# GuildOfWeavers/distaff

Hardware: NVIDIA H100
Metric: prove ms for 2^20-step trace (default 120-bit ProofOptions) (lower is better)
Workload: dtype u128 (128-bit prime field) + u32 (blake3)

## Files before the change

distaff_b200/csrc/air.cu:

```cuda
#define DG_MUL_CALL 1
#include "air.h"
#include "air_constants.h"

namespace dg {

__constant__ fe c_sponge_mds[16], c_sponge_inv_mds[16], c_hasher_mds[36], c_hasher_inv_mds[36];

void air_upload_constants(Context &c) {
    if (c.air_consts) return;
    auto conv = [](const unsigned long long (*t)[2], int n, std::vector<fe> &out) {
        out.resize(n);
        for (int i = 0; i < n; i++) out[i] = fe_make(t[i][0], t[i][1]);
    };
    std::vector<fe> v;
    conv(DG_SPONGE_MDS, 16, v);      DG_CUDA(cudaMemcpyToSymbol(c_sponge_mds, v.data(), 16 * sizeof(fe)));
    conv(DG_SPONGE_INV_MDS, 16, v);  DG_CUDA(cudaMemcpyToSymbol(c_sponge_inv_mds, v.data(), 16 * sizeof(fe)));
    conv(DG_HASHER_MDS, 36, v);      DG_CUDA(cudaMemcpyToSymbol(c_hasher_mds, v.data(), 36 * sizeof(fe)));
    conv(DG_HASHER_INV_MDS, 36, v);  DG_CUDA(cudaMemcpyToSymbol(c_hasher_inv_mds, v.data(), 36 * sizeof(fe)));
    c.air_consts = true;
}

__device__ __forceinline__ fe tw_pow(const TwiddleRef &t, unsigned long long e) {
    unsigned ee = (unsigned)(e & (unsigned long long)t.mask);
    return fe_mul(t.lo[ee & ((1u << t.lo_bits) - 1u)], t.hi[ee >> t.lo_bits]);
}

#ifdef DG_AIR_NOSYNC
#define DG_STEP()
#else
#define DG_STEP() __syncthreads()
#endif

template <int W>
__device__ __forceinline__ void matvec(const fe *m, fe *s) {
    fe r[W];
#pragma unroll
    for (int i = 0; i < W; i++) {
        r[i] = fe_dot<W>(m + i * W, s);
        DG_STEP();
    }
#pragma unroll
    for (int i = 0; i < W; i++) s[i] = r[i];
}

#define ONE fe_make(1, 0)
#define ZERO fe_make(0, 0)
__device__ __forceinline__ fe bnot(fe v) { return fe_sub(ONE, v); }
__device__ __forceinline__ fe is_bin(fe v) { return fe_sub(fe_sqr(v), v); }

enum { G2 = 0, G3 = 1, G4 = 2, G6 = 3, G7 = 4, G8 = 5 };

struct Acc {
    fe_wide res;
    fe adj[6];
    const fe *cA, *cB;
    bool nonzero, first;
    __device__ __forceinline__ void fold(int idx, int group, fe v) {
        if (first) { wide_set(res, DG_MUL_WIDE(v, cA[idx])); first = false; }
        else wide_add(res, DG_MUL_WIDE(v, cA[idx]));
        adj[group] = fe_add(adj[group], fe_mul(v, cB[idx]));
        nonzero = nonzero || !fe_is_zero(v);
    }
};

template <int BLOCK, int MIN_BLOCKS>
__global__ void __launch_bounds__(BLOCK, MIN_BLOCKS) constraint_eval_kernel(const AirParams P) {
    const unsigned long long n = 1ULL << P.log_n;
    const unsigned long long total = n * (unsigned long long)P.num_c8;
    unsigned long long gid = (unsigned long long)blockIdx.x * blockDim.x + threadIdx.x;
    const bool live = gid < total;
    if (!live) gid = total - 1;
    const unsigned long long c8_local = gid >> P.log_n, k = gid & (n - 1);
    const unsigned long long c8 = c8_local + P.c8_base;
    const unsigned long long s = (k << 3) + c8;
    const int stride = 1 << (P.log_blowup - 3);
    const unsigned long long N = P.col_stride;
    const unsigned long long lde_index = s * (unsigned long long)stride;
    const fe *cur_p = P.ext + (c8_local * stride) * n + k;
    const fe *nxt_p = P.ext + (c8_local * stride) * n + ((k + 1) & (n - 1));
    const unsigned long long out_idx = (c8_local << P.log_n) + k;

    const int cl = P.cl, ll = P.ll, sl = P.sl;
    const int ctx_off = 15, loop_off = 15 + P.ctx_depth, stk_off = 15 + P.ctx_depth + P.loop_depth;

    fe cur_dec[15], nxt_dec[15];
    fe c_ctx[16], n_ctx[16], c_loop[8], n_loop[8], o[32], nw[32];
    {
        for (int j = 0; j < 15; j++) cur_dec[j] = cur_p[(unsigned long long)j * N];
        for (int j = 0; j < P.ctx_depth; j++) c_ctx[j] = cur_p[(unsigned long long)(ctx_off + j) * N];
        for (int j = 0; j < P.loop_depth; j++) c_loop[j] = cur_p[(unsigned long long)(loop_off + j) * N];
        for (int j = 0; j < P.stack_depth; j++) o[j] = cur_p[(unsigned long long)(stk_off + j) * N];
        for (int j = P.ctx_depth; j < cl; j++) c_ctx[j] = ZERO;
        for (int j = P.loop_depth; j < ll; j++) c_loop[j] = ZERO;
        for (int j = P.stack_depth; j < sl; j++) o[j] = ZERO;
        for (int j = 0; j < 15; j++) nxt_dec[j] = nxt_p[(unsigned long long)j * N];
        for (int j = 0; j < P.ctx_depth; j++) n_ctx[j] = nxt_p[(unsigned long long)(ctx_off + j) * N];
        for (int j = P.ctx_depth; j < cl; j++) n_ctx[j] = ZERO;
        for (int j = 0; j < P.loop_depth; j++) n_loop[j] = nxt_p[(unsigned long long)(loop_off + j) * N];
        for (int j = P.loop_depth; j < ll; j++) n_loop[j] = ZERO;
        for (int j = 0; j < P.stack_depth; j++) nw[j] = nxt_p[(unsigned long long)(stk_off + j) * N];
        for (int j = P.stack_depth; j < sl; j++) nw[j] = ZERO;
    }

    DG_STEP();
    const fe op_counter = cur_dec[0];
    const fe *sp = cur_dec + 1, *cf = cur_dec + 5, *ld = cur_dec + 8, *hd = cur_dec + 13;
    const fe *nsp = nxt_dec + 1, *ncf = nxt_dec + 5;
    fe cff[8], ldf[32], hdf[4];
    {
        fe a3 = fe_mul(cf[0], cf[1]);
        fe a1 = fe_sub(cf[0], a3), a2 = fe_sub(cf[1], a3), a0 = fe_sub(bnot(cf[0]), a2);
        cff[4] = fe_mul(a0, cf[2]); cff[5] = fe_mul(a1, cf[2]); cff[6] = fe_mul(a2, cf[2]); cff[7] = fe_mul(a3, cf[2]);
        cff[0] = fe_sub(a0, cff[4]); cff[1] = fe_sub(a1, cff[5]); cff[2] = fe_sub(a2, cff[6]); cff[3] = fe_sub(a3, cff[7]);
    }
    fe hdf_raw0;
    {
        hdf[3] = fe_mul(hd[0], hd[1]);
        hdf[1] = fe_sub(hd[0], hdf[3]); hdf[2] = fe_sub(hd[1], hdf[3]); hdf[0] = fe_sub(bnot(hd[0]), hdf[2]);
        hdf_raw0 = hdf[0];
        hdf[0] = fe_mul(hdf[0], ld[0]);
    }
    fe next_void;
    {
        fe a3 = fe_mul(ncf[0], ncf[1]);
        next_void = fe_mul(a3, ncf[2]);
    }

    Acc acc;
    acc.first = true;
#pragma unroll
    for (int g = 0; g < 6; g++) acc.adj[g] = ZERO;
    acc.cA = P.coefA; acc.cB = P.coefB; acc.nonzero = false;

    const fe *per = P.per_override ? P.per_override : P.periodic + (s & 127ULL) * 23;

    DG_STEP();
    {
        fe cf_sum = ZERO, ld_prod = ONE, hd_prod = ONE;
#pragma unroll
        for (int i = 0; i < 3; i++) { acc.fold(i, G2, is_bin(cf[i])); cf_sum = fe_add(cf_sum, cf[i]); }
#pragma unroll
        for (int i = 0; i < 5; i++) { acc.fold(3 + i, G2, is_bin(ld[i])); ld_prod = fe_mul(ld_prod, ld[i]); }
#pragma unroll
        for (int i = 0; i < 2; i++) { acc.fold(8 + i, G2, is_bin(hd[i])); hd_prod = fe_mul(hd_prod, hd[i]); }
        fe is_hacc = cff[0];
        fe hacc_t = fe_mul(fe_add(op_counter, ONE), is_hacc);
        fe rest_t = fe_mul(op_counter, bnot(is_hacc));
        acc.fold(10, G3, fe_sub(fe_add(hacc_t, rest_t), nxt_dec[0]));
        acc.fold(11, G8, fe_mul(op_counter, fe_mul(bnot(ld_prod), bnot(hd_prod))));
        acc.fold(12, G8, fe_mul(cf_sum, bnot(fe_mul(ld_prod, hd_prod))));
        acc.fold(13, G6, fe_mul(cff[7], bnot(next_void)));
        fe prefix = fe_add(fe_add(cff[1], cff[4]), fe_add(cff[5], cff[6]));
        fe align = fe_mul(prefix, per[8 + 1]);
        align = fe_add(align, fe_mul(fe_add(cff[2], cff[3]), per[8 + 0]));
        align = fe_add(align, fe_mul(hdf[0], per[8 + 2]));
        acc.fold(14, G4, align);
    }

    DG_STEP();
    {
        fe r_sp[4], r_img;
        {
            fe f = cff[0];
            fe op_value = fe_mul(nw[0], hdf[0]);
            fe os[4], ns[4];
#pragma unroll
            for (int i = 0; i < 4; i++) os[i] = fe_cube(fe_add(sp[i], per[i]));
            DG_STEP();
            matvec<4>(c_sponge_mds, os);
            fe opc = ld[0];
            opc = fe_add(opc, fe_mul_small(ld[1], 2)); opc = fe_add(opc, fe_mul_small(ld[2], 4));
            opc = fe_add(opc, fe_mul_small(ld[3], 8)); opc = fe_add(opc, fe_mul_small(ld[4], 16));
            opc = fe_add(opc, fe_mul_small(hd[0], 32)); opc = fe_add(opc, fe_mul_small(hd[1], 64));
            os[0] = fe_add(os[0], opc);
            os[1] = fe_add(os[1], op_value);
#pragma unroll
            for (int i = 0; i < 4; i++) ns[i] = nsp[i];
            matvec<4>(c_sponge_inv_mds, ns);
#pragma unroll
            for (int i = 0; i < 4; i++) ns[i] = fe_sub(fe_cube(ns[i]), per[4 + i]);
#pragma unroll
            for (int i = 0; i < 4; i++) r_sp[i] = fe_mul(f, fe_sub(os[i], ns[i]));
        }
        DG_STEP();
        {
            fe fclr = fe_add(fe_add(cff[1], cff[4]), cff[5]);
#pragma unroll
            for (int i = 0; i < 4; i++) r_sp[i] = fe_add(r_sp[i], fe_mul(fclr, nsp[i]));
        }
        DG_STEP();
        {
            fe ft = cff[2], ff = cff[3], fb = fe_add(ft, ff);
            r_sp[0] = fe_add(r_sp[0], fe_mul(fb, fe_sub(c_ctx[0], nsp[0])));
            r_sp[1] = fe_add(r_sp[1], fe_mul(ft, fe_sub(sp[0], nsp[1])));
            r_sp[2] = fe_add(r_sp[2], fe_mul(ff, fe_sub(sp[0], nsp[2])));
            r_sp[3] = fe_add(r_sp[3], fe_mul(fb, nsp[3]));
        }
        {
            fe fk = fe_add(cff[6], cff[7]);
#pragma unroll
            for (int i = 0; i < 4; i++) r_sp[i] = fe_add(r_sp[i], fe_mul(fk, fe_sub(sp[i], nsp[i])));
        }
        acc.fold(15, G6, r_sp[0]); acc.fold(16, G7, r_sp[1]); acc.fold(17, G6, r_sp[2]); acc.fold(18, G6, r_sp[3]);
        r_img = fe_mul(fe_add(cff[5], cff[6]), fe_sub(sp[0], c_loop[0]));
        acc.fold(19, G4, r_img);

        DG_STEP();
        {
            fe f_push = fe_add(cff[1], cff[4]), f_pop = fe_add(cff[2], cff[3]), f_copy = fe_add(fe_add(cff[5], cff[6]), cff[7]);
            for (int i = 0; i < cl; i++) {
                fe v = fe_mul(f_copy, fe_sub(c_ctx[i], n_ctx[i]));
                if (i == 0) v = fe_add(v, fe_mul(f_push, fe_sub(sp[0], n_ctx[0])));
// ... 215 lines not shown
    }
    if (live) P.t_ev[out_idx] = t_res;
}

template <int BLOCK, int MIN_BLOCKS, bool STAGE_DEC, bool WIDE_SLOTS>
__global__ void __launch_bounds__(BLOCK, MIN_BLOCKS) constraint_eval_smem_kernel(const AirParams P) {
    extern __shared__ __align__(16) unsigned char air_smem[];
    fe *s_rows = reinterpret_cast<fe *>(air_smem);
    constexpr int PITCH = BLOCK + 1;
    const int tid = threadIdx.x;
    const unsigned long long n = 1ULL << P.log_n;
    const unsigned long long total = n * (unsigned long long)P.num_c8;
    unsigned long long gid = (unsigned long long)blockIdx.x * blockDim.x + threadIdx.x;
    const bool live = gid < total;
    if (!live) gid = total - 1;
    const unsigned long long c8_local = gid >> P.log_n, k = gid & (n - 1);
    const unsigned long long c8 = c8_local + P.c8_base;
    const unsigned long long s = (k << 3) + c8;
    const int stride = 1 << (P.log_blowup - 3);
    const unsigned long long N = P.col_stride;
    const unsigned long long lde_index = s * (unsigned long long)stride;
    const fe *cur_p = P.ext + (c8_local * stride) * n + k;
    const fe *nxt_p = P.ext + (c8_local * stride) * n + ((k + 1) & (n - 1));
    const unsigned long long out_idx = (c8_local << P.log_n) + k;

    const int cl = P.cl, ll = P.ll, sl = P.sl;
    const int ctx_off = 15, loop_off = 15 + P.ctx_depth, stk_off = 15 + P.ctx_depth + P.loop_depth;

    constexpr int S0 = STAGE_DEC ? 0 : 15;
    {
        const int staged = P.w - S0;
        for (int j = 0; j < staged; j++) s_rows[j * PITCH + tid] = cur_p[(unsigned long long)(S0 + j) * N];
        if (tid < staged) {
            const unsigned long long gl = (unsigned long long)blockIdx.x * BLOCK + (BLOCK - 1);
            const unsigned long long cl8 = gl >> P.log_n, kl = gl & (n - 1);
            s_rows[tid * PITCH + BLOCK] = P.ext[(unsigned long long)(S0 + tid) * N + (cl8 * stride) * n + ((kl + 1) & (n - 1))];
        }
    }
    fe cur_dec[STAGE_DEC ? 1 : 15], nxt_dec[STAGE_DEC ? 1 : 15];
    if constexpr (!STAGE_DEC) {
#pragma unroll
        for (int j = 0; j < 15; j++) { cur_dec[j] = cur_p[(unsigned long long)j * N]; nxt_dec[j] = nxt_p[(unsigned long long)j * N]; }
    }
    __syncthreads();
#define DCUR(j) (STAGE_DEC ? s_rows[(j) * PITCH + tid] : cur_dec[STAGE_DEC ? 0 : (j)])
#define DNXT(j) (STAGE_DEC ? s_rows[(j) * PITCH + tid + 1] : nxt_dec[STAGE_DEC ? 0 : (j)])
#define SCOL(col, nx) s_rows[((col) - S0) * PITCH + tid + (nx)]
#define C_CTX(i) (((i) < P.ctx_depth) ? SCOL(ctx_off + (i), 0) : ZERO)
#define N_CTX(i) (((i) < P.ctx_depth) ? SCOL(ctx_off + (i), 1) : ZERO)
#define C_LOOP(i) (((i) < P.loop_depth) ? SCOL(loop_off + (i), 0) : ZERO)
#define N_LOOP(i) (((i) < P.loop_depth) ? SCOL(loop_off + (i), 1) : ZERO)
#define O(i) (((i) < P.stack_depth) ? SCOL(stk_off + (i), 0) : ZERO)
#define NW(i) (((i) < P.stack_depth) ? SCOL(stk_off + (i), 1) : ZERO)

    DG_STEP();
    const fe op_counter = DCUR(0);
#define sp(i) DCUR(1 + (i))
#define cf(i) DCUR(5 + (i))
#define ld(i) DCUR(8 + (i))
#define hd(i) DCUR(13 + (i))
#define nsp(i) DNXT(1 + (i))
#define ncf(i) DNXT(5 + (i))
    fe cff[8], ldf[32], hdf[4];
    {
        fe a3 = fe_mul(cf(0), cf(1));
        fe a1 = fe_sub(cf(0), a3), a2 = fe_sub(cf(1), a3), a0 = fe_sub(bnot(cf(0)), a2);
        cff[4] = fe_mul(a0, cf(2)); cff[5] = fe_mul(a1, cf(2)); cff[6] = fe_mul(a2, cf(2)); cff[7] = fe_mul(a3, cf(2));
        cff[0] = fe_sub(a0, cff[4]); cff[1] = fe_sub(a1, cff[5]); cff[2] = fe_sub(a2, cff[6]); cff[3] = fe_sub(a3, cff[7]);
    }
    fe hdf_raw0;
    {
        hdf[3] = fe_mul(hd(0), hd(1));
        hdf[1] = fe_sub(hd(0), hdf[3]); hdf[2] = fe_sub(hd(1), hdf[3]); hdf[0] = fe_sub(bnot(hd(0)), hdf[2]);
        hdf_raw0 = hdf[0];
        hdf[0] = fe_mul(hdf[0], ld(0));
    }
    fe next_void;
    {
        fe a3 = fe_mul(ncf(0), ncf(1));
        next_void = fe_mul(a3, ncf(2));
    }

    Acc acc;
    acc.first = true;
#pragma unroll
    for (int g = 0; g < 6; g++) acc.adj[g] = ZERO;
    acc.cA = P.coefA; acc.cB = P.coefB; acc.nonzero = false;

    const fe *per = P.per_override ? P.per_override : P.periodic + (s & 127ULL) * 23;

    DG_STEP();
    {
        fe cf_sum = ZERO, ld_prod = ONE, hd_prod = ONE;
#pragma unroll
        for (int i = 0; i < 3; i++) { acc.fold(i, G2, is_bin(cf(i))); cf_sum = fe_add(cf_sum, cf(i)); }
#pragma unroll
        for (int i = 0; i < 5; i++) { acc.fold(3 + i, G2, is_bin(ld(i))); ld_prod = fe_mul(ld_prod, ld(i)); }
#pragma unroll
        for (int i = 0; i < 2; i++) { acc.fold(8 + i, G2, is_bin(hd(i))); hd_prod = fe_mul(hd_prod, hd(i)); }
        fe is_hacc = cff[0];
        fe hacc_t = fe_mul(fe_add(op_counter, ONE), is_hacc);
        fe rest_t = fe_mul(op_counter, bnot(is_hacc));
        acc.fold(10, G3, fe_sub(fe_add(hacc_t, rest_t), DNXT(0)));
        acc.fold(11, G8, fe_mul(op_counter, fe_mul(bnot(ld_prod), bnot(hd_prod))));
        acc.fold(12, G8, fe_mul(cf_sum, bnot(fe_mul(ld_prod, hd_prod))));
        acc.fold(13, G6, fe_mul(cff[7], bnot(next_void)));
        fe prefix = fe_add(fe_add(cff[1], cff[4]), fe_add(cff[5], cff[6]));
        fe align = fe_mul(prefix, per[8 + 1]);
        align = fe_add(align, fe_mul(fe_add(cff[2], cff[3]), per[8 + 0]));
        align = fe_add(align, fe_mul(hdf[0], per[8 + 2]));
        acc.fold(14, G4, align);
    }

    DG_STEP();
    {
        fe r_sp[4], r_img;
        {
            fe f = cff[0];
            fe op_value = fe_mul(NW(0), hdf[0]);
            fe os[4], ns[4];
#pragma unroll
            for (int i = 0; i < 4; i++) os[i] = fe_cube(fe_add(sp(i), per[i]));
            DG_STEP();
            matvec<4>(c_sponge_mds, os);
            fe opc = ld(0);
            opc = fe_add(opc, fe_mul_small(ld(1), 2)); opc = fe_add(opc, fe_mul_small(ld(2), 4));
            opc = fe_add(opc, fe_mul_small(ld(3), 8)); opc = fe_add(opc, fe_mul_small(ld(4), 16));
            opc = fe_add(opc, fe_mul_small(hd(0), 32)); opc = fe_add(opc, fe_mul_small(hd(1), 64));
            os[0] = fe_add(os[0], opc);
            os[1] = fe_add(os[1], op_value);
#pragma unroll
            for (int i = 0; i < 4; i++) ns[i] = nsp(i);
            matvec<4>(c_sponge_inv_mds, ns);
#pragma unroll
            for (int i = 0; i < 4; i++) ns[i] = fe_sub(fe_cube(ns[i]), per[4 + i]);
#pragma unroll
            for (int i = 0; i < 4; i++) r_sp[i] = fe_mul(f, fe_sub(os[i], ns[i]));
        }
        DG_STEP();
        {
            fe fclr = fe_add(fe_add(cff[1], cff[4]), cff[5]);
#pragma unroll
            for (int i = 0; i < 4; i++) r_sp[i] = fe_add(r_sp[i], fe_mul(fclr, nsp(i)));
        }
        DG_STEP();
        {
            fe ft = cff[2], ff = cff[3], fb = fe_add(ft, ff);
            r_sp[0] = fe_add(r_sp[0], fe_mul(fb, fe_sub(C_CTX(0), nsp(0))));
            r_sp[1] = fe_add(r_sp[1], fe_mul(ft, fe_sub(sp(0), nsp(1))));
            r_sp[2] = fe_add(r_sp[2], fe_mul(ff, fe_sub(sp(0), nsp(2))));
            r_sp[3] = fe_add(r_sp[3], fe_mul(fb, nsp(3)));
        }
        {
            fe fk = fe_add(cff[6], cff[7]);
#pragma unroll
            for (int i = 0; i < 4; i++) r_sp[i] = fe_add(r_sp[i], fe_mul(fk, fe_sub(sp(i), nsp(i))));
        }
        acc.fold(15, G6, r_sp[0]); acc.fold(16, G7, r_sp[1]); acc.fold(17, G6, r_sp[2]); acc.fold(18, G6, r_sp[3]);
        r_img = fe_mul(fe_add(cff[5], cff[6]), fe_sub(sp(0), C_LOOP(0)));
        acc.fold(19, G4, r_img);

        DG_STEP();
        {
            fe f_push = fe_add(cff[1], cff[4]), f_pop = fe_add(cff[2], cff[3]), f_copy = fe_add(fe_add(cff[5], cff[6]), cff[7]);
            for (int i = 0; i < cl; i++) {
                fe v = fe_mul(f_copy, fe_sub(C_CTX(i), N_CTX(i)));
                if (i == 0) v = fe_add(v, fe_mul(f_push, fe_sub(sp(0), N_CTX(0))));
// ... 169 lines not shown
            fe c = O(4), nc = bnot(c);
            ev[0] = fe_add(ev[0], fe_mul(f_choose2, fe_sub(NW(0), fe_add(fe_mul(c, O(0)), fe_mul(nc, O(2))))));
            ev[1] = fe_add(ev[1], fe_mul(f_choose2, fe_sub(NW(1), fe_add(fe_mul(c, O(1)), fe_mul(nc, O(3))))));
            ev[0] = fe_add(ev[0], fe_mul(f_cswap2, fe_sub(NW(0), fe_add(fe_mul(c, O(2)), fe_mul(nc, O(0))))));
            ev[1] = fe_add(ev[1], fe_mul(f_cswap2, fe_sub(NW(1), fe_add(fe_mul(c, O(3)), fe_mul(nc, O(1))))));
            ev[2] = fe_add(ev[2], fe_mul(f_cswap2, fe_sub(NW(2), fe_add(fe_mul(c, O(0)), fe_mul(nc, O(2))))));
            ev[3] = fe_add(ev[3], fe_mul(f_cswap2, fe_sub(NW(3), fe_add(fe_mul(c, O(1)), fe_mul(nc, O(3))))));
        }
        DG_STEP();
        {
            fe bit = NW(0);
            ev[0] = fe_add(ev[0], fe_mul(f_binacc, is_bin(bit)));
            ev[1] = fe_add(ev[1], fe_mul(f_binacc, NW(1)));
            ev[2] = fe_add(ev[2], fe_mul(f_binacc, fe_sub(NW(2), fe_mul_small(O(2), 2))));
            ev[3] = fe_add(ev[3], fe_mul(f_binacc, fe_sub(NW(3), fe_add(O(3), fe_mul(bit, O(2))))));
        }
        DG_STEP();
        {
            fe xb = NW(1), yb = NW(2), not_set = NW(3);
            fe bit_gt = fe_mul(xb, bnot(yb)), bit_lt = fe_mul(yb, bnot(xb));
            fe gt = fe_add(O(4), fe_mul(bit_gt, not_set)), lt = fe_add(O(5), fe_mul(bit_lt, not_set));
            fe p2 = O(0);
            fe x_acc = fe_add(O(7), fe_mul(xb, p2)), y_acc = fe_add(O(6), fe_mul(yb, p2));
            fe nsc = fe_mul(bnot(O(5)), bnot(O(4)));
            ev[0] = fe_add(ev[0], fe_mul(f_cmp, is_bin(xb)));
            ev[1] = fe_add(ev[1], fe_mul(f_cmp, is_bin(yb)));
            ev[2] = fe_add(ev[2], fe_mul(f_cmp, fe_sub(NW(4), gt)));
            ev[3] = fe_add(ev[3], fe_mul(f_cmp, fe_sub(NW(5), lt)));
            ev[4] = fe_add(ev[4], fe_mul(f_cmp, fe_sub(NW(6), y_acc)));
            ev[5] = fe_add(ev[5], fe_mul(f_cmp, fe_sub(NW(7), x_acc)));
            ev[6] = fe_add(ev[6], fe_mul(f_cmp, fe_sub(not_set, nsc)));
            ev[7] = fe_add(ev[7], fe_mul(f_cmp, fe_sub(fe_mul_small(NW(0), 2), p2)));
        }
        DG_STEP();
        {
            fe os[6], ns[6];
#pragma unroll
            for (int q = 0; q < 6; q++) os[q] = fe_cube(fe_add(O(q), per[11 + q]));
            matvec<6>(c_hasher_mds, os);
#pragma unroll
            for (int q = 0; q < 6; q++) ns[q] = NW(q);
            matvec<6>(c_hasher_inv_mds, ns);
#pragma unroll
            for (int q = 0; q < 6; q++) ns[q] = fe_sub(fe_cube(ns[q]), per[11 + 6 + q]);
#pragma unroll
            for (int q = 0; q < 6; q++) ev[q] = fe_add(ev[q], fe_mul(f_rescr, fe_sub(ns[q], os[q])));
        }
#pragma unroll
        for (int i = 0; i < 8; i++)
            if (i < P.stack_depth) acc.fold(base + 2 + i, G7, ev[i]);
    }

    DG_STEP();
    fe t_res = DG_REDUCE_WIDE(acc.res);
#pragma unroll
    for (int g = 0; g < 6; g++) t_res = fe_add(t_res, fe_mul(acc.adj[g], P.xpow_override ? P.xpow_override[g] : tw_pow(P.twN, lde_index * P.inc[g])));
    if (!P.verify_mode && c8 == 0 && k != n - 1) {
        if (acc.nonzero && live) atomicExch(P.violation, (unsigned)(k + 1));
        t_res = ZERO;
    }
    if (live) P.t_ev[out_idx] = t_res;
}

#undef DCUR
#undef DNXT
#undef SCOL
#undef C_CTX
#undef N_CTX
#undef C_LOOP
#undef N_LOOP
#undef O
#undef NW
#undef sp
#undef cf
#undef ld
#undef hd
#undef nsp
#undef ncf

void launch_constraint_eval(Context &c, const AirParams &P) {
    air_upload_constants(c);
    const unsigned long long E = (unsigned long long)P.num_c8 << P.log_n;
    static int variant = -1;
    if (variant < 0) { const char *e = getenv("DG_AIR_CFG"); variant = e ? atoi(e) : 7; }
#define DG_AIR_LAUNCH(BLOCK, MINB) constraint_eval_kernel<BLOCK, MINB><<<(unsigned)((E + BLOCK - 1) / BLOCK), BLOCK, 0, c.stream>>>(P)
#define DG_AIR_LAUNCH_SMEM(BLOCK, MINB, DEC, WIDE)                                                                                         \
    do {                                                                                                                             \
        const size_t smem = (size_t)(P.w - ((DEC) ? 0 : 15)) * (BLOCK + 1) * sizeof(fe);                                             \
        auto k = constraint_eval_smem_kernel<BLOCK, MINB, DEC, WIDE>;                                                                      \
        set_func_smem(c, (const void *)k, smem);                                                                                     \
        k<<<(unsigned)(E / BLOCK), BLOCK, smem, c.stream>>>(P);                                                                      \
    } while (0)
    int v = variant;
    const unsigned long long n = 1ULL << P.log_n;
    if (v < 5 || v > 7) v = 1;
    if (v >= 5 && (n < 128 || (size_t)P.w * 129 * sizeof(fe) > 200 * 1024)) v = 1;
    switch (v) {
        case 5: DG_AIR_LAUNCH_SMEM(128, 4, false, false); break;
        case 6: DG_AIR_LAUNCH_SMEM(128, 4, true, false); break;
        case 7: DG_AIR_LAUNCH_SMEM(128, 4, true, true); break;
        default: DG_AIR_LAUNCH(128, 4); break;
    }
    c.launches++;
    DG_CUDA(cudaGetLastError());
}

}
```

distaff_b200/csrc/air.h:

```cpp
#pragma once
#include "common.cuh"

namespace dg {

struct AirParams {
    int w, ctx_depth, loop_depth, stack_depth;
    int cl, ll, sl;
    int log_n, log_blowup;
    const fe *ext;
    unsigned long long col_stride;
    int c8_base, num_c8;
    fe *t_ev;
    const fe *periodic;
    const fe *coefA, *coefB;
    TwiddleRef twN;
    unsigned long long inc[6];
    unsigned *violation;
    int verify_mode;
    const fe *per_override;
    const fe *xpow_override;
};

void launch_constraint_eval(Context &c, const AirParams &P);

}
```

Before: 95.79.

## Split constraint evaluation into three phase kernels with smaller staged column sets

Replaces the single monolithic constraint-evaluation kernel with three sequential phase kernels: decoder/sponge/context/loop, stack shifts and ops, and hasher/comparison. Each phase stages only the columns it needs into shared memory, which lowers per-kernel register pressure and shared memory use and should raise occupancy. Partial sums are accumulated into t_ev across phases. Boundary rows needing cross-phase values go through a temporary ev0 buffer, and wide (unreduced) accumulators are kept for the adjustment groups. The cost is extra launches, re-reading some columns and the output buffer, plus a device allocation per call.

```diff
diff --git a/distaff_b200/csrc/air.cu b/distaff_b200/csrc/air.cu
--- a/distaff_b200/csrc/air.cu
+++ b/distaff_b200/csrc/air.cu
@@ -1,5 +1,5 @@
 #define DG_MUL_CALL 1
-#include "air.h"
+#include "air_eval.cuh"
 #include "air_constants.h"
 
 namespace dg {
@@ -19,49 +19,6 @@
     conv(DG_HASHER_INV_MDS, 36, v);  DG_CUDA(cudaMemcpyToSymbol(c_hasher_inv_mds, v.data(), 36 * sizeof(fe)));
     c.air_consts = true;
 }
-
-__device__ __forceinline__ fe tw_pow(const TwiddleRef &t, unsigned long long e) {
-    unsigned ee = (unsigned)(e & (unsigned long long)t.mask);
-    return fe_mul(t.lo[ee & ((1u << t.lo_bits) - 1u)], t.hi[ee >> t.lo_bits]);
-}
-
-#ifdef DG_AIR_NOSYNC
-#define DG_STEP()
-#else
-#define DG_STEP() __syncthreads()
-#endif
-
-template <int W>
-__device__ __forceinline__ void matvec(const fe *m, fe *s) {
-    fe r[W];
-#pragma unroll
-    for (int i = 0; i < W; i++) {
-        r[i] = fe_dot<W>(m + i * W, s);
-        DG_STEP();
-    }
-#pragma unroll
-    for (int i = 0; i < W; i++) s[i] = r[i];
-}
-
-#define ONE fe_make(1, 0)
-#define ZERO fe_make(0, 0)
-__device__ __forceinline__ fe bnot(fe v) { return fe_sub(ONE, v); }
-__device__ __forceinline__ fe is_bin(fe v) { return fe_sub(fe_sqr(v), v); }
-
-enum { G2 = 0, G3 = 1, G4 = 2, G6 = 3, G7 = 4, G8 = 5 };
-
-struct Acc {
-    fe_wide res;
-    fe adj[6];
-    const fe *cA, *cB;
-    bool nonzero, first;
-    __device__ __forceinline__ void fold(int idx, int group, fe v) {
-        if (first) { wide_set(res, DG_MUL_WIDE(v, cA[idx])); first = false; }
-        else wide_add(res, DG_MUL_WIDE(v, cA[idx]));
-        adj[group] = fe_add(adj[group], fe_mul(v, cB[idx]));
-        nonzero = nonzero || !fe_is_zero(v);
-    }
-};
 
 template <int BLOCK, int MIN_BLOCKS>
 __global__ void __launch_bounds__(BLOCK, MIN_BLOCKS) constraint_eval_kernel(const AirParams P) {
@@ -127,7 +84,7 @@
     }
 
     Acc acc;
-    acc.first = true;
+    acc.first = true; acc.combine = true;
 #pragma unroll
     for (int g = 0; g < 6; g++) acc.adj[g] = ZERO;
     acc.cA = P.coefA; acc.cB = P.coefB; acc.nonzero = false;
@@ -509,7 +466,7 @@
     }
 
     Acc acc;
-    acc.first = true;
+    acc.first = true; acc.combine = true;
 #pragma unroll
     for (int g = 0; g < 6; g++) acc.adj[g] = ZERO;
     acc.cA = P.coefA; acc.cB = P.coefB; acc.nonzero = false;
@@ -845,26 +802,24 @@
     air_upload_constants(c);
     const unsigned long long E = (unsigned long long)P.num_c8 << P.log_n;
     static int variant = -1;
-    if (variant < 0) { const char *e = getenv("DG_AIR_CFG"); variant = e ? atoi(e) : 7; }
-#define DG_AIR_LAUNCH(BLOCK, MINB) constraint_eval_kernel<BLOCK, MINB><<<(unsigned)((E + BLOCK - 1) / BLOCK), BLOCK, 0, c.stream>>>(P)
-#define DG_AIR_LAUNCH_SMEM(BLOCK, MINB, DEC, WIDE)                                                                                         \
-    do {                                                                                                                             \
-        const size_t smem = (size_t)(P.w - ((DEC) ? 0 : 15)) * (BLOCK + 1) * sizeof(fe);                                             \
-        auto k = constraint_eval_smem_kernel<BLOCK, MINB, DEC, WIDE>;                                                                      \
-        set_func_smem(c, (const void *)k, smem);                                                                                     \
-        k<<<(unsigned)(E / BLOCK), BLOCK, smem, c.stream>>>(P);                                                                      \
-    } while (0)
+    if (variant < 0) { const char *e = getenv("DG_AIR_CFG"); variant = e ? atoi(e) : 8; }
     int v = variant;
     const unsigned long long n = 1ULL << P.log_n;
-    if (v < 5 || v > 7) v = 1;
-    if (v >= 5 && (n < 128 || (size_t)P.w * 129 * sizeof(fe) > 200 * 1024)) v = 1;
-    switch (v) {
-        case 5: DG_AIR_LAUNCH_SMEM(128, 4, false, false); break;
-        case 6: DG_AIR_LAUNCH_SMEM(128, 4, true, false); break;
-        case 7: DG_AIR_LAUNCH_SMEM(128, 4, true, true); break;
-        default: DG_AIR_LAUNCH(128, 4); break;
-    }
-    c.launches++;
+    if (v != 7 && v != 8) v = 1;
+    if (v == 7 && (P.verify_mode || n < 128 || (size_t)P.w * 129 * sizeof(fe) > 200 * 1024)) v = 1;
+    if (v == 8 && !constraint_phases_fit(P)) v = 1;
+    if (v == 8) {
+        launch_constraint_phases(c, P);
+    } else if (v == 7) {
+        const size_t smem = (size_t)P.w * 129 * sizeof(fe);
+        auto k = constraint_eval_smem_kernel<128, 4, true, true>;
+        set_func_smem(c, (const void *)k, smem);
+        k<<<(unsigned)(E / 128), 128, smem, c.stream>>>(P);
+        c.launches++;
+    } else {
+        constraint_eval_kernel<128, 4><<<(unsigned)((E + 127) / 128), 128, 0, c.stream>>>(P);
+        c.launches++;
+    }
     DG_CUDA(cudaGetLastError());
 }
 
diff --git a/distaff_b200/csrc/air.h b/distaff_b200/csrc/air.h
--- a/distaff_b200/csrc/air.h
+++ b/distaff_b200/csrc/air.h
@@ -22,5 +22,7 @@
 };
 
 void launch_constraint_eval(Context &c, const AirParams &P);
+bool constraint_phases_fit(const AirParams &P);
+void launch_constraint_phases(Context &c, const AirParams &P);
 
 }
diff --git a/distaff_b200/csrc/air_eval.cuh b/distaff_b200/csrc/air_eval.cuh
--- /dev/null
+++ b/distaff_b200/csrc/air_eval.cuh
@@ -0,0 +1,75 @@
+#pragma once
+#include "air.h"
+
+namespace dg {
+
+extern __constant__ fe c_sponge_mds[16], c_sponge_inv_mds[16], c_hasher_mds[36], c_hasher_inv_mds[36];
+
+__device__ __forceinline__ fe tw_pow(const TwiddleRef &t, unsigned long long e) {
+    unsigned ee = (unsigned)(e & (unsigned long long)t.mask);
+    return fe_mul(t.lo[ee & ((1u << t.lo_bits) - 1u)], t.hi[ee >> t.lo_bits]);
+}
+
+#ifdef DG_AIR_NOSYNC
+#define DG_STEP()
+#else
+#define DG_STEP() __syncthreads()
+#endif
+
+template <int W>
+__device__ __forceinline__ void matvec(const fe *m, fe *s) {
+    fe r[W];
+#pragma unroll
+    for (int i = 0; i < W; i++) {
+        r[i] = fe_dot<W>(m + i * W, s);
+        DG_STEP();
+    }
+#pragma unroll
+    for (int i = 0; i < W; i++) s[i] = r[i];
+}
+
+#define ONE fe_make(1, 0)
+#define ZERO fe_make(0, 0)
+__device__ __forceinline__ fe bnot(fe v) { return fe_sub(ONE, v); }
+__device__ __forceinline__ fe is_bin(fe v) { return fe_sub(fe_sqr(v), v); }
+
+enum { G2 = 0, G3 = 1, G4 = 2, G6 = 3, G7 = 4, G8 = 5 };
+
+struct Acc {
+    fe_wide res;
+    fe adj[6];
+    const fe *cA, *cB;
+    bool nonzero, first, combine;
+    __device__ __forceinline__ void fold(int idx, int group, fe v) {
+        if (combine) {
+            if (first) { wide_set(res, DG_MUL_WIDE(v, cA[idx])); first = false; }
+            else wide_add(res, DG_MUL_WIDE(v, cA[idx]));
+            adj[group] = fe_add(adj[group], fe_mul(v, cB[idx]));
+        }
+        nonzero = nonzero || !fe_is_zero(v);
+    }
+};
+
+struct AccWide {
+    fe_wide res, adj[6];
+    const fe *cA, *cB;
+    bool nonzero, combine;
+    __device__ __forceinline__ void init(const fe *a, const fe *b, bool comb) {
+#pragma unroll
+        for (int i = 0; i < 9; i++) {
+            res.r[i] = 0;
+#pragma unroll
+            for (int g = 0; g < 6; g++) adj[g].r[i] = 0;
+        }
+        cA = a; cB = b; nonzero = false; combine = comb;
+    }
+    __device__ __forceinline__ void fold(int idx, int group, fe v) {
+        if (combine) {
+            wide_add(res, DG_MUL_WIDE(v, cA[idx]));
+            wide_add(adj[group], DG_MUL_WIDE(v, cB[idx]));
+        }
+        nonzero = nonzero || !fe_is_zero(v);
+    }
+};
+
+}
diff --git a/distaff_b200/csrc/air_phase.cu b/distaff_b200/csrc/air_phase.cu
--- /dev/null
+++ b/distaff_b200/csrc/air_phase.cu
@@ -0,0 +1,479 @@
+#define DG_MUL_CALL 1
+#include "air_eval.cuh"
+
+namespace dg {
+
+namespace {
+
+constexpr int PH_BLOCK = 128;
+constexpr int PH_PITCH = PH_BLOCK + 1;
+
+template <int PHASE> struct PhaseCols {
+    static constexpr int a0 = PHASE == 0 ? 0 : PHASE == 1 ? 6 : 13;
+    static constexpr int na = 15 - a0;
+};
+template <int PHASE>
+__host__ __device__ __forceinline__ void phase_range(const AirParams &P, int &b0, int &b1) {
+    const int stk_off = 15 + P.ctx_depth + P.loop_depth;
+    if (PHASE == 0) { b0 = 15; b1 = stk_off + (P.stack_depth > 0 ? 1 : 0); }
+    else if (PHASE == 1) { b0 = stk_off; b1 = P.w; }
+    else { b0 = stk_off; b1 = stk_off + (P.stack_depth < 8 ? P.stack_depth : 8); }
+}
+template <int PHASE>
+size_t phase_smem(const AirParams &P) {
+    int b0, b1;
+    phase_range<PHASE>(P, b0, b1);
+    return (size_t)(PhaseCols<PHASE>::na + b1 - b0) * PH_PITCH * sizeof(fe);
+}
+
+template <int PHASE, int GROUPS>
+__device__ __forceinline__ void phase_finish(const AirParams &P, const AccWide &acc, unsigned long long c8, unsigned long long k, unsigned long long n,
+                                             unsigned long long lde_index, unsigned long long out_idx, bool live) {
+    fe t = ZERO;
+    if (acc.combine) {
+        t = DG_REDUCE_WIDE(acc.res);
+#pragma unroll
+        for (int g = 0; g < 6; g++)
+            if (GROUPS & (1 << g)) t = fe_add(t, fe_mul(DG_REDUCE_WIDE(acc.adj[g]), tw_pow(P.twN, lde_index * P.inc[g])));
+    }
+    if (c8 == 0 && k != n - 1) {
+        if (acc.nonzero && live) atomicExch(P.violation, (unsigned)(k + 1));
+        t = ZERO;
+    }
+    if (live) P.t_ev[out_idx] = PHASE == 0 ? t : fe_add(P.t_ev[out_idx], t);
+}
+
+template <int PHASE, int MINB>
+__global__ void __launch_bounds__(PH_BLOCK, MINB) constraint_phase_kernel(const AirParams P, fe *ev0) {
+    extern __shared__ __align__(16) unsigned char air_smem[];
+    fe *s_rows = reinterpret_cast<fe *>(air_smem);
+    constexpr int BLOCK = PH_BLOCK, PITCH = PH_PITCH;
+    constexpr int A0 = PhaseCols<PHASE>::a0, NA = PhaseCols<PHASE>::na;
+    const int tid = threadIdx.x;
+    const unsigned long long n = 1ULL << P.log_n;
+    const unsigned long long total = n * (unsigned long long)P.num_c8;
+    unsigned long long gid = (unsigned long long)blockIdx.x * blockDim.x + threadIdx.x;
+    const bool live = gid < total;
+    if (!live) gid = total - 1;
+    const unsigned long long c8_local = gid >> P.log_n, k = gid & (n - 1);
+    const unsigned long long c8 = c8_local + P.c8_base;
+    const unsigned long long s = (k << 3) + c8;
+    const int stride = 1 << (P.log_blowup - 3);
+    const unsigned long long N = P.col_stride;
+    const unsigned long long lde_index = s * (unsigned long long)stride;
+    const fe *cur_p = P.ext + (c8_local * stride) * n + k;
+    const unsigned long long out_idx = (c8_local << P.log_n) + k;
+
+    const int cl = P.cl, ll = P.ll;
+    const int ctx_off = 15, loop_off = 15 + P.ctx_depth, stk_off = 15 + P.ctx_depth + P.loop_depth;
+    int B0, B1;
+    phase_range<PHASE>(P, B0, B1);
+    {
+        const int staged = NA + B1 - B0;
+        for (int j = 0; j < staged; j++) {
+            const int col = j < NA ? A0 + j : B0 + (j - NA);
+            s_rows[j * PITCH + tid] = cur_p[(unsigned long long)col * N];
+        }
+        if (tid < staged) {
+            const int col = tid < NA ? A0 + tid : B0 + (tid - NA);
+            const unsigned long long gl = (unsigned long long)blockIdx.x * BLOCK + (BLOCK - 1);
+            const unsigned long long cl8 = gl >> P.log_n, kl = gl & (n - 1);
+            s_rows[tid * PITCH + BLOCK] = P.ext[(unsigned long long)col * N + (cl8 * stride) * n + ((kl + 1) & (n - 1))];
+        }
+    }
+    __syncthreads();
+#define DCUR(j) s_rows[((j) - A0) * PITCH + tid]
+#define DNXT(j) s_rows[((j) - A0) * PITCH + tid + 1]
+#define SCOL(col, nx) s_rows[(NA + (col) - B0) * PITCH + tid + (nx)]
+#define C_CTX(i) (((i) < P.ctx_depth) ? SCOL(ctx_off + (i), 0) : ZERO)
+#define N_CTX(i) (((i) < P.ctx_depth) ? SCOL(ctx_off + (i), 1) : ZERO)
+#define C_LOOP(i) (((i) < P.loop_depth) ? SCOL(loop_off + (i), 0) : ZERO)
+#define N_LOOP(i) (((i) < P.loop_depth) ? SCOL(loop_off + (i), 1) : ZERO)
+#define O(i) (((i) < P.stack_depth) ? SCOL(stk_off + (i), 0) : ZERO)
+#define NW(i) (((i) < P.stack_depth) ? SCOL(stk_off + (i), 1) : ZERO)
+#define sp(i) DCUR(1 + (i))
+#define cf(i) DCUR(5 + (i))
+#define ld(i) DCUR(8 + (i))
+#define hd(i) DCUR(13 + (i))
+#define nsp(i) DNXT(1 + (i))
+#define ncf(i) DNXT(5 + (i))
+
+    AccWide acc;
+    {
+        const unsigned long long k_last = ((unsigned long long)blockIdx.x * BLOCK + (BLOCK - 1)) & (n - 1);
+        acc.init(P.coefA, P.coefB, c8 != 0 || k_last == n - 1);
+    }
+    const fe *per = P.periodic + (s & 127ULL) * 23;
+    const int base = 20 + cl + ll;
+
+    if constexpr (PHASE == 0) {
+        const fe op_counter = DCUR(0);
+        fe cff[8], push_flag, next_void;
+        {
+            fe a3 = fe_mul(cf(0), cf(1));
+            fe a1 = fe_sub(cf(0), a3), a2 = fe_sub(cf(1), a3), a0 = fe_sub(bnot(cf(0)), a2);
+            cff[4] = fe_mul(a0, cf(2)); cff[5] = fe_mul(a1, cf(2)); cff[6] = fe_mul(a2, cf(2)); cff[7] = fe_mul(a3, cf(2));
+            cff[0] = fe_sub(a0, cff[4]); cff[1] = fe_sub(a1, cff[5]); cff[2] = fe_sub(a2, cff[6]); cff[3] = fe_sub(a3, cff[7]);
+        }
+        {
+            fe h3 = fe_mul(hd(0), hd(1));
+            push_flag = fe_mul(fe_sub(bnot(hd(0)), fe_sub(hd(1), h3)), ld(0));
+        }
+        {
+            fe a3 = fe_mul(ncf(0), ncf(1));
+            next_void = fe_mul(a3, ncf(2));
+        }
+        DG_STEP();
+        {
+            fe cf_sum = ZERO, ld_prod = ONE, hd_prod = ONE;
+#pragma unroll
+            for (int i = 0; i < 3; i++) { acc.fold(i, G2, is_bin(cf(i))); cf_sum = fe_add(cf_sum, cf(i)); }
+#pragma unroll
+            for (int i = 0; i < 5; i++) { acc.fold(3 + i, G2, is_bin(ld(i))); ld_prod = fe_mul(ld_prod, ld(i)); }
+#pragma unroll
+            for (int i = 0; i < 2; i++) { acc.fold(8 + i, G2, is_bin(hd(i))); hd_prod = fe_mul(hd_prod, hd(i)); }
+            fe is_hacc = cff[0];
+            fe hacc_t = fe_mul(fe_add(op_counter, ONE), is_hacc);
+            fe rest_t = fe_mul(op_counter, bnot(is_hacc));
+            acc.fold(10, G3, fe_sub(fe_add(hacc_t, rest_t), DNXT(0)));
+            acc.fold(11, G8, fe_mul(op_counter, fe_mul(bnot(ld_prod), bnot(hd_prod))));
+            acc.fold(12, G8, fe_mul(cf_sum, bnot(fe_mul(ld_prod, hd_prod))));
+            acc.fold(13, G6, fe_mul(cff[7], bnot(next_void)));
+            fe prefix = fe_add(fe_add(cff[1], cff[4]), fe_add(cff[5], cff[6]));
+            fe align = fe_mul(prefix, per[8 + 1]);
+            align = fe_add(align, fe_mul(fe_add(cff[2], cff[3]), per[8 + 0]));
+            align = fe_add(align, fe_mul(push_flag, per[8 + 2]));
+            acc.fold(14, G4, align);
+        }
+        DG_STEP();
+        {
+            fe r_sp[4];
+            {
+                fe f = cff[0];
+                fe op_value = fe_mul(NW(0), push_flag);
+                fe os[4], ns[4];
+#pragma unroll
+                for (int i = 0; i < 4; i++) os[i] = fe_cube(fe_add(sp(i), per[i]));
+                DG_STEP();
+                matvec<4>(c_sponge_mds, os);
+                fe opc = ld(0);
+                opc = fe_add(opc, fe_mul_small(ld(1), 2)); opc = fe_add(opc, fe_mul_small(ld(2), 4));
+                opc = fe_add(opc, fe_mul_small(ld(3), 8)); opc = fe_add(opc, fe_mul_small(ld(4), 16));
+                opc = fe_add(opc, fe_mul_small(hd(0), 32)); opc = fe_add(opc, fe_mul_small(hd(1), 64));
+                os[0] = fe_add(os[0], opc);
+                os[1] = fe_add(os[1], op_value);
+#pragma unroll
+                for (int i = 0; i < 4; i++) ns[i] = nsp(i);
+                matvec<4>(c_sponge_inv_mds, ns);
+#pragma unroll
+                for (int i = 0; i < 4; i++) ns[i] = fe_sub(fe_cube(ns[i]), per[4 + i]);
+#pragma unroll
+                for (int i = 0; i < 4; i++) r_sp[i] = fe_mul(f, fe_sub(os[i], ns[i]));
+            }
+            DG_STEP();
+            {
+                fe fclr = fe_add(fe_add(cff[1], cff[4]), cff[5]);
+#pragma unroll
+                for (int i = 0; i < 4; i++) r_sp[i] = fe_add(r_sp[i], fe_mul(fclr, nsp(i)));
+            }
+            {
+                fe ft = cff[2], ff = cff[3], fb = fe_add(ft, ff);
+                r_sp[0] = fe_add(r_sp[0], fe_mul(fb, fe_sub(C_CTX(0), nsp(0))));
+                r_sp[1] = fe_add(r_sp[1], fe_mul(ft, fe_sub(sp(0), nsp(1))));
+                r_sp[2] = fe_add(r_sp[2], fe_mul(ff, fe_sub(sp(0), nsp(2))));
+                r_sp[3] = fe_add(r_sp[3], fe_mul(fb, nsp(3)));
+            }
+            {
+                fe fk = fe_add(cff[6], cff[7]);
+#pragma unroll
+                for (int i = 0; i < 4; i++) r_sp[i] = fe_add(r_sp[i], fe_mul(fk, fe_sub(sp(i), nsp(i))));
+            }
+            acc.fold(15, G6, r_sp[0]); acc.fold(16, G7, r_sp[1]); acc.fold(17, G6, r_sp[2]); acc.fold(18, G6, r_sp[3]);
+            acc.fold(19, G4, fe_mul(fe_add(cff[5], cff[6]), fe_sub(sp(0), C_LOOP(0))));
+
+            DG_STEP();
+            {
+                fe f_push = fe_add(cff[1], cff[4]), f_pop = fe_add(cff[2], cff[3]), f_copy = fe_add(fe_add(cff[5], cff[6]), cff[7]);
+#pragma unroll 1
+                for (int i = 0; i < cl; i++) {
+                    fe v = fe_mul(f_copy, fe_sub(C_CTX(i), N_CTX(i)));
+                    if (i == 0) v = fe_add(v, fe_mul(f_push, fe_sub(sp(0), N_CTX(0))));
+                    else v = fe_add(v, fe_mul(f_push, fe_sub(C_CTX(i - 1), N_CTX(i))));
+                    if (i < cl - 1) v = fe_add(v, fe_mul(f_pop, fe_sub(C_CTX(i + 1), N_CTX(i))));
+                    else v = fe_add(v, fe_mul(f_pop, N_CTX(i)));
+                    acc.fold(20 + i, G4, v);
+                }
+            }
+            DG_STEP();
+            {
+                fe f_copy = fe_add(fe_add(fe_add(cff[1], cff[2]), fe_add(cff[3], cff[5])), cff[7]);
+                fe f_rs = cff[4], f_ls = cff[6];
+#pragma unroll 1
+                for (int i = 0; i < ll; i++) {
+                    fe v = fe_mul(f_copy, fe_sub(C_LOOP(i), N_LOOP(i)));
+                    if (i >= 1) v = fe_add(v, fe_mul(f_rs, fe_sub(C_LOOP(i - 1), N_LOOP(i))));
+                    if (i < ll - 1) v = fe_add(v, fe_mul(f_ls, fe_sub(C_LOOP(i + 1), N_LOOP(i))));
+                    else v = fe_add(v, fe_mul(f_ls, N_LOOP(i)));
+                    acc.fold(20 + cl + i, G4, v);
+                }
+            }
+        }
+        DG_STEP();
+        phase_finish<0, 0x3f>(P, acc, c8, k, n, lde_index, out_idx, live);
+    } else if constexpr (PHASE == 1) {
+        fe ldf[32], hdf[4], hdf_raw0;
+        {
+            hdf[3] = fe_mul(hd(0), hd(1));
+            hdf[1] = fe_sub(hd(0), hdf[3]); hdf[2] = fe_sub(hd(1), hdf[3]); hdf[0] = fe_sub(bnot(hd(0)), hdf[2]);
+            hdf_raw0 = hdf[0];
+            hdf[0] = fe_mul(hdf[0], ld(0));
+        }
+        {
+            fe n0 = bnot(ld(0));
+            ldf[3] = fe_mul(ld(0), ld(1));
+            ldf[1] = fe_sub(ld(0), ldf[3]);
+            ldf[0] = fe_sub(n0, fe_sub(ld(1), ldf[3]));
+            ldf[2] = fe_mul(n0, cf(1));
+#pragma unroll
+            for (int i = 0; i < 4; i++) { ldf[4 + i] = fe_mul(ldf[i], ld(2)); ldf[i] = fe_sub(ldf[i], ldf[4 + i]); }
+#pragma unroll
+            for (int i = 0; i < 8; i++) { ldf[8 + i] = fe_mul(ldf[i], ld(3)); ldf[i] = fe_sub(ldf[i], ldf[8 + i]); }
+            DG_STEP();
+#pragma unroll
+            for (int i = 0; i < 16; i++) { ldf[16 + i] = fe_mul(ldf[i], ld(4)); ldf[i] = fe_sub(ldf[i], ldf[16 + i]); }
+        }
+        DG_STEP();
+        const fe begin_flag = fe_mul(ldf[0], hdf_raw0), noop_flag = fe_mul(ldf[31], hdf[3]);
+        ldf[0] = fe_mul(ldf[0], hd(0));
+        DG_STEP();
+        const int L = P.sl;
+        const fe f_assert = ldf[0], f_asserteq = ldf[1], f_eq = ldf[2], f_drop = ldf[3], f_drop4 = ldf[4], f_choose = ldf[5],
+                 f_choose2 = ldf[6], f_cswap2 = ldf[7], f_add = ldf[8], f_mul = ldf[9], f_and = ldf[10], f_or = ldf[11], f_inv = ldf[12],
+                 f_neg = ldf[13], f_not = ldf[14], f_read = ldf[16], f_read2 = ldf[17], f_dup = ldf[18], f_dup2 = ldf[19],
+                 f_dup4 = ldf[20], f_pad2 = ldf[21], f_swap = ldf[24], f_swap2 = ldf[25], f_swap4 = ldf[26], f_roll4 = ldf[27],
+                 f_roll8 = ldf[28], f_binacc = ldf[29];
+        const fe f_push = hdf[0], f_cmp = hdf[1], f_rescr = hdf[2];
+        {
+            fe aux0, aux1;
+            aux0 = fe_mul(f_assert, fe_sub(ONE, O(0)));
+            aux0 = fe_add(aux0, fe_mul(f_asserteq, fe_sub(O(0), O(1))));
+            fe b0 = is_bin(O(0)), b1 = is_bin(O(1));
+            fe f_ao = fe_add(f_and, f_or);
+            aux0 = fe_add(aux0, fe_mul(fe_add(f_not, f_ao), b0));
+            aux1 = fe_mul(f_ao, b1);
+            fe diff = fe_sub(O(1), O(2));
+            aux0 = fe_add(aux0, fe_mul(f_eq, fe_mul(NW(0), diff)));
+            aux0 = fe_add(aux0, fe_mul(f_choose, is_bin(O(2))));
+            aux0 = fe_add(aux0, fe_mul(fe_add(f_choose2, f_cswap2), is_bin(O(4))));
+            acc.fold(base, G7, aux0);
+            acc.fold(base + 1, G7, aux1);
+        }
+        DG_STEP();
+        fe ev[8];
+        const fe f_copy0 = fe_add(begin_flag, noop_flag);
+        const fe f_copy1 = fe_add(fe_add(f_inv, f_neg), f_not);
+        const fe f_copy2 = f_swap;
+        const fe f_copy4 = fe_add(fe_add(f_swap2, f_roll4), f_binacc);
+        const fe f_copy6 = f_rescr;
+        const fe f_copy8 = fe_add(fe_add(f_swap4, f_roll8), f_cmp);
+        const fe f_rs1 = fe_add(fe_add(f_read, f_dup), f_push);
+        const fe f_rs2 = fe_add(fe_add(f_read2, f_dup2), f_pad2);
+        const fe f_rs4 = f_dup4;
+        const fe f_ls1_0 = fe_add(f_assert, f_drop);
+        const fe f_ls1_1 = fe_add(fe_add(f_add, f_mul), fe_add(f_and, f_or));
+        const fe f_ls2_0 = f_asserteq;
+        const fe f_ls2_1 = fe_add(f_eq, f_choose);
+        const fe f_ls2_4 = f_cswap2;
+        const fe f_ls4_0 = f_drop4;
+        const fe f_ls4_2 = f_choose2;
+        auto slot_value = [&](const int i, const fe fc, const fe fl1, const fe fl2, const fe fl4) -> fe {
+            const fe nwi = NW(i);
+            fe_wide acc7;
+            wide_set(acc7, DG_MUL_WIDE(fc, fe_sub(O(i), nwi)));
+            if (i >= 1) wide_add(acc7, DG_MUL_WIDE(f_rs1, fe_sub(O(i - 1), nwi)));
+            if (i >= 2) wide_add(acc7, DG_MUL_WIDE(f_rs2, fe_sub(O(i - 2), nwi)));
+            if (i >= 4) wide_add(acc7, DG_MUL_WIDE(f_rs4, fe_sub(O(i - 4), nwi)));
+            wide_add(acc7, DG_MUL_WIDE(fl1, (i < L - 1) ? fe_sub(O(i + 1), nwi) : nwi));
+            wide_add(acc7, DG_MUL_WIDE(fl2, (i < L - 2) ? fe_sub(O(i + 2), nwi) : nwi));
+            wide_add(acc7, DG_MUL_WIDE(fl4, (i < L - 4) ? fe_sub(O(i + 4), nwi) : nwi));
+            return DG_REDUCE_WIDE(acc7);
+        };
+        fe fc_hi, fl1_hi, fl2_hi, fl4_hi;
+        {
+            fe fc = f_copy0, fl1 = f_ls1_0, fl2 = f_ls2_0, fl4 = f_ls4_0;
+#pragma unroll
+            for (int i = 0; i < 8; i++) {
+                if (i == 1) { fc = fe_add(fc, f_copy1); fl1 = fe_add(fl1, f_ls1_1); fl2 = fe_add(fl2, f_ls2_1); }
+                if (i == 2) { fc = fe_add(fc, f_copy2); fl4 = fe_add(fl4, f_ls4_2); }
+                if (i == 4) { fc = fe_add(fc, f_copy4); fl2 = fe_add(fl2, f_ls2_4); }
+                if (i == 6) fc = fe_add(fc, f_copy6);
+                ev[i] = slot_value(i, fc, fl1, fl2, fl4);
+                if (i & 1) DG_STEP();
+            }
+            fc_hi = fe_add(fc, f_copy8); fl1_hi = fl1; fl2_hi = fl2; fl4_hi = fl4;
+        }
+#pragma unroll 1
+        for (int i = 8; i < L; i++) {
+            acc.fold(base + 2 + i, G7, slot_value(i, fc_hi, fl1_hi, fl2_hi, fl4_hi));
+            DG_STEP();
+        }
+        DG_STEP();
+        ev[0] = fe_add(ev[0], fe_mul(fe_add(fe_add(f_dup, f_dup2), f_dup4), fe_sub(NW(0), O(0))));
+        ev[1] = fe_add(ev[1], fe_mul(fe_add(f_dup2, f_dup4), fe_sub(NW(1), O(1))));
+        ev[2] = fe_add(ev[2], fe_mul(f_dup4, fe_sub(NW(2), O(2))));
+        ev[3] = fe_add(ev[3], fe_mul(f_dup4, fe_sub(NW(3), O(3))));
+        ev[0] = fe_add(ev[0], fe_mul(f_pad2, NW(0)));
+        ev[1] = fe_add(ev[1], fe_mul(f_pad2, NW(1)));
+        ev[0] = fe_add(ev[0], fe_mul(f_swap, fe_add(fe_sub(NW(0), O(1)), fe_sub(NW(1), O(0)))));
+        DG_STEP();
+        ev[0] = fe_add(ev[0], fe_mul(f_swap2, fe_sub(NW(0), O(2)))); ev[1] = fe_add(ev[1], fe_mul(f_swap2, fe_sub(NW(1), O(3))));
+        ev[2] = fe_add(ev[2], fe_mul(f_swap2, fe_sub(NW(2), O(0)))); ev[3] = fe_add(ev[3], fe_mul(f_swap2, fe_sub(NW(3), O(1))));
+#pragma unroll
+        for (int q = 0; q < 4; q++) {
+            ev[q] = fe_add(ev[q], fe_mul(f_swap4, fe_sub(NW(q), O(4 + q))));
+            ev[4 + q] = fe_add(ev[4 + q], fe_mul(f_swap4, fe_sub(NW(4 + q), O(q))));
+        }
+        DG_STEP();
+        ev[0] = fe_add(ev[0], fe_mul(f_roll4, fe_sub(NW(0), O(3))));
+#pragma unroll
+        for (int q = 1; q < 4; q++) ev[q] = fe_add(ev[q], fe_mul(f_roll4, fe_sub(NW(q), O(q - 1))));
+        ev[0] = fe_add(ev[0], fe_mul(f_roll8, fe_sub(NW(0), O(7))));
+#pragma unroll
+        for (int q = 1; q < 8; q++) ev[q] = fe_add(ev[q], fe_mul(f_roll8, fe_sub(NW(q), O(q - 1))));
+        DG_STEP();
+        {
+            fe prod = fe_mul(O(0), O(1));
+            fe v = fe_mul(f_add, fe_sub(NW(0), fe_add(O(0), O(1))));
+            v = fe_add(v, fe_mul(fe_add(f_mul, f_and), fe_sub(NW(0), prod)));
+            v = fe_add(v, fe_mul(f_inv, fe_sub(ONE, fe_mul(NW(0), O(0)))));
+            v = fe_add(v, fe_mul(f_neg, fe_add(NW(0), O(0))));
+            v = fe_add(v, fe_mul(f_not, fe_sub(NW(0), bnot(O(0)))));
+            v = fe_add(v, fe_mul(f_or, fe_sub(NW(0), bnot(fe_mul(bnot(O(0)), bnot(O(1)))))));
+            v = fe_add(v, fe_mul(f_eq, fe_sub(NW(0), bnot(fe_mul(fe_sub(O(1), O(2)), O(0))))));
+            {
+                fe c = O(2);
+                v = fe_add(v, fe_mul(f_choose, fe_sub(NW(0), fe_add(fe_mul(c, O(0)), fe_mul(bnot(c), O(1))))));
+            }
+            ev[0] = fe_add(ev[0], v);
+        }
+        DG_STEP();
+        {
+            fe c = O(4), nc = bnot(c);
+            ev[0] = fe_add(ev[0], fe_mul(f_choose2, fe_sub(NW(0), fe_add(fe_mul(c, O(0)), fe_mul(nc, O(2))))));
+            ev[1] = fe_add(ev[1], fe_mul(f_choose2, fe_sub(NW(1), fe_add(fe_mul(c, O(1)), fe_mul(nc, O(3))))));
+            ev[0] = fe_add(ev[0], fe_mul(f_cswap2, fe_sub(NW(0), fe_add(fe_mul(c, O(2)), fe_mul(nc, O(0))))));
+            ev[1] = fe_add(ev[1], fe_mul(f_cswap2, fe_sub(NW(1), fe_add(fe_mul(c, O(3)), fe_mul(nc, O(1))))));
+            ev[2] = fe_add(ev[2], fe_mul(f_cswap2, fe_sub(NW(2), fe_add(fe_mul(c, O(0)), fe_mul(nc, O(2))))));
+            ev[3] = fe_add(ev[3], fe_mul(f_cswap2, fe_sub(NW(3), fe_add(fe_mul(c, O(1)), fe_mul(nc, O(3))))));
+        }
+        DG_STEP();
+        {
+            fe bit = NW(0);
+            ev[0] = fe_add(ev[0], fe_mul(f_binacc, is_bin(bit)));
+            ev[1] = fe_add(ev[1], fe_mul(f_binacc, NW(1)));
+            ev[2] = fe_add(ev[2], fe_mul(f_binacc, fe_sub(NW(2), fe_mul_small(O(2), 2))));
+            ev[3] = fe_add(ev[3], fe_mul(f_binacc, fe_sub(NW(3), fe_add(O(3), fe_mul(bit, O(2))))));
+        }
+#pragma unroll
+        for (int i = 0; i < 8; i++) {
+            if (i < P.stack_depth) {
+                if (c8 == 0) { if (live) ev0[(unsigned long long)i * n + k] = ev[i]; }
+                else acc.fold(base + 2 + i, G7, ev[i]);
+            }
+        }
+        DG_STEP();
+        phase_finish<1, 1 << G7>(P, acc, c8, k, n, lde_index, out_idx, live);
+    } else {
+        fe f_cmp, f_rescr;
+        {
+            fe h3 = fe_mul(hd(0), hd(1));
+            f_cmp = fe_sub(hd(0), h3); f_rescr = fe_sub(hd(1), h3);
+        }
+        fe ev[8];
+        {
+            fe xb = NW(1), yb = NW(2), not_set = NW(3);
+            fe bit_gt = fe_mul(xb, bnot(yb)), bit_lt = fe_mul(yb, bnot(xb));
+            fe gt = fe_add(O(4), fe_mul(bit_gt, not_set)), lt = fe_add(O(5), fe_mul(bit_lt, not_set));
+            fe p2 = O(0);
+            fe x_acc = fe_add(O(7), fe_mul(xb, p2)), y_acc = fe_add(O(6), fe_mul(yb, p2));
+            fe nsc = fe_mul(bnot(O(5)), bnot(O(4)));
+            ev[0] = fe_mul(f_cmp, is_bin(xb));
+            ev[1] = fe_mul(f_cmp, is_bin(yb));
+            ev[2] = fe_mul(f_cmp, fe_sub(NW(4), gt));
+            ev[3] = fe_mul(f_cmp, fe_sub(NW(5), lt));
+            ev[4] = fe_mul(f_cmp, fe_sub(NW(6), y_acc));
+            ev[5] = fe_mul(f_cmp, fe_sub(NW(7), x_acc));
+            ev[6] = fe_mul(f_cmp, fe_sub(not_set, nsc));
+            ev[7] = fe_mul(f_cmp, fe_sub(fe_mul_small(NW(0), 2), p2));
+        }
+        DG_STEP();
+        {
+            fe os[6], ns[6];
+#pragma unroll
+            for (int q = 0; q < 6; q++) os[q] = fe_cube(fe_add(O(q), per[11 + q]));
+            matvec<6>(c_hasher_mds, os);
+#pragma unroll
+            for (int q = 0; q < 6; q++) ns[q] = NW(q);
+            matvec<6>(c_hasher_inv_mds, ns);
+#pragma unroll
+            for (int q = 0; q < 6; q++) ns[q] = fe_sub(fe_cube(ns[q]), per[11 + 6 + q]);
+#pragma unroll
+            for (int q = 0; q < 6; q++) ev[q] = fe_add(ev[q], fe_mul(f_rescr, fe_sub(ns[q], os[q])));
+        }
+#pragma unroll
+        for (int i = 0; i < 8; i++) {
+            if (i < P.stack_depth) {
+                fe v = ev[i];
+                if (c8 == 0) v = fe_add(v, ev0[(unsigned long long)i * n + k]);
+                acc.fold(base + 2 + i, G7, v);
+            }
+        }
+        DG_STEP();
+        phase_finish<2, 1 << G7>(P, acc, c8, k, n, lde_index, out_idx, live);
+    }
+#undef DCUR
+#undef DNXT
+#undef SCOL
+#undef C_CTX
+#undef N_CTX
+#undef C_LOOP
+#undef N_LOOP
+#undef O
+#undef NW
+#undef sp
+#undef cf
+#undef ld
+#undef hd
+#undef nsp
+#undef ncf
+}
+
+template <int PHASE>
+void launch_phase(Context &c, const AirParams &P, fe *ev0, unsigned long long E) {
+    constexpr int MINB = PHASE == 2 ? 5 : 4;
+    const size_t smem = phase_smem<PHASE>(P);
+    auto kern = constraint_phase_kernel<PHASE, MINB>;
+    set_func_smem(c, (const void *)kern, smem);
+    kern<<<(unsigned)(E / PH_BLOCK), PH_BLOCK, smem, c.stream>>>(P, ev0);
+    c.launches++;
+}
+
+}
+
+bool constraint_phases_fit(const AirParams &P) {
+    const size_t limit = 200 * 1024;
+    return !P.verify_mode && P.log_n >= 7 && phase_smem<0>(P) <= limit && phase_smem<1>(P) <= limit && phase_smem<2>(P) <= limit;
+}
+
+void launch_constraint_phases(Context &c, const AirParams &P) {
+    const unsigned long long n = 1ULL << P.log_n, E = (unsigned long long)P.num_c8 << P.log_n;
+    DevBuf ev0;
+    if (P.c8_base == 0) ev0.alloc(n * 8 * sizeof(fe));
+    launch_phase<0>(c, P, ev0.as<fe>(), E);
+    if (c.mark) c.mark("3.eval.p0");
+    launch_phase<1>(c, P, ev0.as<fe>(), E);
+    if (c.mark) c.mark("3.eval.p1");
+    launch_phase<2>(c, P, ev0.as<fe>(), E);
+}
+
+}
```

Result: no change. 94.90, median of 6 (-0.9%).
